# Ryo1011gd/ParticleMethod_FSI

Hardware: AMD Instinct MI355X
Metric: particle-steps/sec + achieved HBM GB/s, dam-break, 1/2/4/8 MI355X (higher is better)
Workload: dtype f64; 1 GPU; d1m: 3-D dam break (SURVEY 8d D1M, BASELINE configs[1]), 1397200 particles, ~1397200 per GPU; particles=1397200, dim=3, module=dam, parallelism=single

## Files before the change

include/mph_gpu.h:

```cpp
#ifndef MPH_GPU_H_INCLUDED
#define MPH_GPU_H_INCLUDED

#include <stddef.h>

#ifdef __cplusplus
extern "C" {
#endif

#define MPH_TYPE_COUNT 6
#define MPH_MAX_NEIGHBOR_COUNT 512
#define MPH_ABI_VERSION 6

typedef enum MphModule {
    MPH_MODULE_BAR = 0,
    MPH_MODULE_DAM = 1,
    MPH_MODULE_TUREK_HRON = 2,
    MPH_MODULE_ROLLING1 = 3,
    MPH_MODULE_HYDROELASTIC = 4,
    MPH_MODULE_NONE = 5
} MphModule;

typedef enum MphWallMotion {
    MPH_WALL_RIGID = 0,
    MPH_WALL_ROLLING = 1
// ... 227 lines not shown
    const char* unique_id128;
    mph_host_exchange_fn host_fn;
    void* host_user;
    int n_glob;
    const int* ids;
    const double* cuts;
} MphSlabOptions;
int mph_create_slab(MphCtx** ctx, const MphConfig* cfg, int n, const int* property, const double* pos,
                    const double* pos0, const double* vel, int device, const MphSlabOptions* opt);
int mph_slab_window(const MphConfig* cfg, int rank, int nranks, int axis, const double* cuts, double* out2);
int mph_dist_selftest(int device);
int mph_dist_info(const MphCtx* ctx, int* out8);
int mph_dist_overlap(const MphCtx* ctx, double* out5);
int mph_list_stats(MphCtx* ctx, double* mean, int* max);
int mph_list_layout(MphCtx* ctx, long long out6[6]);
int mph_neighbor_rows(MphCtx* ctx, int first, int count, int* counts, int* ids, long long ids_cap);
int mph_owned_count(const MphCtx* ctx);
int mph_owned_ids(MphCtx* ctx, int* out_ids);
int mph_slab_bounds(const MphConfig* cfg, int rank, int nranks, int axis, const double* cuts, double* out3);
int mph_slab_owner(const MphConfig* cfg, int nranks, int axis, const double* cuts, double c);

#ifdef __cplusplus
}
#endif
#endif
```

particlemethod_fsi_amd/csrc/mph_ctx.h:

```cpp
#pragma once

#include <hip/hip_runtime.h>

#include <cstdlib>
#include <string>
#include <thread>
#include <vector>

#include "mph_internal.h"
#include "mph_kernels.h"

struct MphDist {
    int rank = 0, nranks = 1, left = 0, right = 0;
    mph::SlabGeom g{};
    std::vector<double> cuts;
    int cap = 0;
    int n_own = 0;
    mph::DistLayout* lay = nullptr;
    mph::DistLayout* hlay = nullptr;
    int cap_sl = 0, cap_sr = 0, cap_rl = 0, cap_rr = 0;
    size_t region = 0;
    mph::Soa C;
    int* cls = nullptr;
    int* vidx = nullptr;
// ... 58 lines not shown
    std::vector<int> sl_s;
    int* order = nullptr;
    double *vir = nullptr, *vpres = nullptr;
    mph::StructDev Sd;
    std::vector<void*> allocs;
    mph::Launch L;
    bool mon_on = false;
    mph::MonitorDev mon;
    size_t mon_ring_cap = 0;
    int *mon_sorted = nullptr, *mon_map = nullptr;
    double* mon_probes = nullptr;
    long long mon_read = 0;
    double* sample_out = nullptr;
    size_t sample_cap = 0;
    bool a_current = false;
    MphDist* dist = nullptr;
};

#define MPH_HIP_OK(ctx, expr)                                                \
    do {                                                                     \
        hipError_t _e = (expr);                                              \
        if (_e != hipSuccess) return mph::ctx_hip_fail(ctx, _e, #expr);      \
    } while (0)

#define MPH_CK(expr)                   \
    do {                               \
        int _r = (expr);               \
        if (_r != MPH_OK) return _r;   \
    } while (0)

// ... 51 lines not shown
```

particlemethod_fsi_amd/csrc/mph_ctx.hip:

```cpp
#include <hip/hip_runtime.h>

#include <algorithm>
#include <chrono>
#include <cmath>
#include <cstdio>
#include <cstdlib>
#include <cstring>
#include <map>
#include <memory>
#include <string>
#include <vector>

#include "mph_ctx.h"
#include "mph_rows.h"

using namespace mph;

namespace mph {

int ctx_fail(MphCtx* c, int code, const std::string& msg)
{
    if (c) c->err = msg;
    return code;
}
// ... 30 lines not shown
    if (hs.overflow & 4)
        return ctx_fail(c, MPH_ERR_NONFINITE, "non-finite particle position (diverged state)");
    if (hs.overflow & 1)
        return ctx_fail(c, MPH_ERR_NEIGHBOR_OVERFLOW, "a particle has more than 512 neighbours");
    if (hs.overflow & 2) return ctx_fail(c, MPH_ERR_CAPACITY, "a particle moved past a neighbouring slab");
    if (hs.overflow & 64)
        return ctx_fail(c, MPH_ERR_HIP, "cell sort: histogram inconsistent with the keys (placement out of range)");
    return MPH_OK;
}

void ctx_fill_launch(MphCtx* c)
{
    Launch& L = c->L;
    set_uniforms(c->P);
    if (std::getenv("MPH_LIST_FULL") && std::atoi(std::getenv("MPH_LIST_FULL")) == 1) c->P.rlf = 3.0e38f;
    L.P = &c->P;
    L.stream = c->stream;
    const char* bm = std::getenv("MPH_XCD_BAL_MIN");
    L.xcd_bal_min = bm && *bm ? std::atoi(bm) : (1 << 20);
    L.S = &c->Sd;
}

int virial_full_lists(MphCtx* c)
{
    if (c->P.rlf >= 3.0e38f) return MPH_OK;
    DevParams Pf = c->P;
    Pf.rlf = 3.0e38f;
    Launch L = c->L;
    L.P = &Pf;
    L.xcd_bal_min = 0x7fffffff;
    launch_neighbors(L);
    MPH_HIP_OK(c, hipGetLastError());
    return MPH_OK;
}
}

namespace {

void enqueue_step(const Launch& L, bool last, hipEvent_t* ev = nullptr)
{
    if (ev) (void)hipEventRecord(ev[0], L.stream);
    launch_sort(L, 1);
    Launch La = L;
    if (!last) {
        La.dens_a = La.vstrain = La.divp = nullptr;
        if (!L.P->surface) La.gx = La.gy = La.gz = La.pa = nullptr;
    }
    if (ev) {
        launch_neighbors(La);
        (void)hipEventRecord(ev[1], L.stream);
        launch_pass_a(La);
    } else {
        launch_search_pass_a(La);
    }
    if (last) {
        launch_pass_b(L);
    } else {
        Launch Lb = L;
        Lb.force = nullptr;
        Lb.acc = nullptr;
        launch_pass_b(Lb);
    }
    launch_structure(L, last);
    if (ev) (void)hipEventRecord(ev[2], L.stream);
    if (L.mon) launch_monitor(L, *L.mon);
}

int capture(MphCtx* c, int steps, hipGraphExec_t* out, bool store_last = true)
{
    hipGraph_t g = nullptr;
    MPH_HIP_OK(c, hipStreamBeginCapture(c->stream, hipStreamCaptureModeThreadLocal));
    for (int k = 0; k < steps; ++k) enqueue_step(c->L, store_last && k == steps - 1);
    MPH_HIP_OK(c, hipStreamEndCapture(c->stream, &g));
    MPH_HIP_OK(c, hipGraphInstantiate(out, g, nullptr, nullptr, 0));
    MPH_HIP_OK(c, hipGraphDestroy(g));
// ... 448 lines not shown
    for (double* m : {D.F, D.E, D.S})
        MPH_HIP_OK(c, hipMemsetAsync(m, 0, sizeof(double) * 9 * nl, c->stream));
    MPH_HIP_OK(c, hipStreamSynchronize(c->stream));
    return MPH_OK;
}

static int init_first_sums(MphCtx* c)
{
    ctx_fill_launch(c);
    if (c->dist) {
        MPH_CK(dist_alloc(c));
        MPH_CK(dist_init(c));
    } else {
        launch_sort(c->L, 0);
        launch_search_pass_a(c->L);
    }
    MPH_HIP_OK(c, hipGetLastError());
    MPH_HIP_OK(c, hipStreamSynchronize(c->stream));
    DevState hs;
    MPH_HIP_OK(c, hipMemcpy(&hs, c->L.st, kStateHead, hipMemcpyDeviceToHost));
    return ctx_state_status(c, hs);
}

static int ctx_init(MphCtx* c, CreateArgs& a)
{
    MPH_CK(init_check_args(c, a));
    MPH_CK(init_host_state(c, a));
    MPH_CK(init_grid(c, a));
    MPH_CK(init_capacity(c, a));
    MPH_CK(init_alloc(c, a));
// ... 588 lines not shown
    for (long long t = 0; t < waves; ++t) {
        const int J = jump_count(R.hdr[t]);
        jumped += J > 0;
        jumps += J;
        max_jumps = std::max<long long>(max_jumps, J);
    }
    for (int s = 0; s < n; ++s) {
        const int rows = std::min(R.rows[s], kTileRows);
        gap_rows += rows - R.entries(s);
        max_rows = std::max<long long>(max_rows, rows);
    }
    out[0] = waves; out[1] = jumped; out[2] = jumps; out[3] = max_jumps; out[4] = gap_rows; out[5] = max_rows;
    return MPH_OK;
}

int mph_neighbor_rows(MphCtx* c, int first, int count, int* counts, int* ids, long long ids_cap)
{
    if (!c || first < 0 || count < 0 || !counts || (!ids && ids_cap > 0)) return MPH_ERR_ARG;
    MPH_CK(ctx_flush(c));
    if (c->dist) return ctx_fail(c, MPH_ERR_UNSUPPORTED, "mph_neighbor_rows: single contexts only");
    if ((long long)first + count > c->n) return ctx_fail(c, MPH_ERR_ARG, "mph_neighbor_rows: range past the particle count");
    if (!count) return 0;
    MPH_HIP_OK(c, hipSetDevice(c->device));
    const int n = c->n;
    if (c->P.rlf < 3.0e38f)
        return ctx_fail(c, MPH_ERR_UNSUPPORTED, "mph_neighbor_rows: the lists keep only the pairs within the passes' "
                                            "radius (create the context with MPH_LIST_FULL=1 for the reference's lists)");
    std::vector<int> id(n), nv(n);
    MPH_HIP_OK(c, hipMemcpy(id.data(), c->L.A.id, sizeof(int) * n, hipMemcpyDeviceToHost));
    MPH_HIP_OK(c, hipMemcpy(nv.data(), c->L.nbcount, sizeof(int) * n, hipMemcpyDeviceToHost));
// ... 251 lines not shown
```

particlemethod_fsi_amd/csrc/mph_device.h:

```cpp
#pragma once

#include <hip/hip_runtime.h>
#include <hip/hip_ext.h>

#include <climits>
#include <type_traits>

#include "mph_kernels.h"
#include "mph_params.h"

namespace mph {

__device__ __forceinline__ double mod_exact(double x, double w)
{
#pragma clang fp contract(off)
    return x - w * floor(x / w);
}

template <bool FAST>
__device__ __forceinline__ double image_exact(double d, double w, double hw, double w075)
{
#pragma clang fp contract(off)
    const double s = d + hw;
    double m;
// ... 56 lines not shown
__device__ __forceinline__ void rsqrt_pair(double r2, double& r, double& ir)
{
    double y = __builtin_amdgcn_rsq(r2);
    const double e = fma(-(r2 * y), y, 1.0);
    y = fma(0.5 * y, e, y);
    ir = y;
    r = r2 * y;
}

__device__ __forceinline__ int cell_id(const DevParams& P, double x, double y, double z)
{
    const int cx = cell_axis(x, P.corg[0], P.dw[0], P.ginv[0], P.gc[0]);
    const int cy = cell_axis(y, P.corg[1], P.dw[1], P.ginv[1], P.gc[1]);
    const int cz = P.dim == 3 ? cell_axis(z, P.corg[2], P.dw[2], P.ginv[2], P.gc[2]) : 0;
    return cell_index(P, cx, cy, cz);
}

__device__ __forceinline__ bool dev_is_struct(int t) { return t == 2 || t == 3; }
__device__ __forceinline__ bool dev_is_fluid(int t) { return t == 0 || t == 1; }
__device__ __forceinline__ bool dev_is_wall(int t) { return t == 4 || t == 5; }

__device__ __forceinline__ bool wave_search_interior(const DevParams& P, const DevState* st, bool live,
                                                     double x, double y, double z)
{
    const int occ = st->seam_occ[(st->seam_step - 1) & 1];
    const double v[3] = {x, y, z};
    bool in = true;
#pragma unroll
    for (int k = 0; k < 3; ++k) {
        if (k == 2 && P.dim == 2) break;
// ... 209 lines not shown
```

particlemethod_fsi_amd/csrc/mph_kernels.h:

```cpp
#pragma once

#include <hip/hip_runtime.h>

#include "mph_params.h"

namespace mph {

struct StructDev {
    int* orig = nullptr;
    int* slot_of = nullptr;
    int* bidx = nullptr;
    int n_own = 0;
    int n_inner = 0;
    int wo = 0, wi = 0;
    int* ocnt = nullptr;
    int* icnt = nullptr;
    int* eo_nb = nullptr;
    int* ei_nb = nullptr;
    double4* wx0 = nullptr;
    double* L = nullptr;
    double2* lame = nullptr;
    double* inv_rho = nullptr;
    int* clamp = nullptr;
    double4* x0 = nullptr;
// ... 52 lines not shown

struct Launch {
    const DevParams* P = nullptr;
    const DevTables* T = nullptr;
    DevState* st = nullptr;
    hipStream_t stream = nullptr;
    Profiler* prof = nullptr;
    Soa A, B;
    int* dst_of = nullptr;
    int *key = nullptr, *slot = nullptr, *tmp = nullptr, *cnt = nullptr, *start = nullptr, *bsum = nullptr;
    int *nbr = nullptr, *ncount = nullptr, *nbcount = nullptr;
    unsigned long long *lhdr = nullptr, *lgap = nullptr;
    int* wface = nullptr;
    VSrc vsrc;
    int xcd_bal_min = 1 << 20;
    double *pres = nullptr, *gx = nullptr, *gy = nullptr, *gz = nullptr, *pa = nullptr;
    double *dens_a = nullptr, *vstrain = nullptr, *divp = nullptr;
    double4 *fpart = nullptr;
    double4 *rec = nullptr;
    double4 *force = nullptr, *acc = nullptr;
    const StructDev* S = nullptr;
    const MonitorDev* mon = nullptr;
};

struct SampleDev {
    double origin[3], spacing[3];
    int count[3];
    int tile[3];
    int tiles[3];
    int mask;
// ... 51 lines not shown
```

particlemethod_fsi_amd/csrc/mph_list.h:

```cpp
#pragma once

#include "mph_device.h"

namespace mph {

#ifndef MPH_LB
#define MPH_LB 256
#endif
constexpr int kWB = MPH_LB / 64;
__device__ __forceinline__ int list_blocks(int n) { return (n + MPH_LB - 1) / MPH_LB; }

constexpr int kWaveCost = 16;

__device__ __forceinline__ int list_block(const DevState* st, int n, bool rev = false)
{
    const int nb = list_blocks(n);
    const int b = blockIdx.x;
    if (st) {
        const int* fr = st->xcd_frac;
        const int cap = gridDim.x >> 3;
        const int j = b & 7;
        bool ok = fr[0] == 0 && fr[8] == 65536;
        int lo = 0, mine_lo = 0, mine_c = 0;
        for (int x = 0; x < 8; ++x) {
            const int hi = (int)(((long long)fr[x + 1] * nb) >> 16);
            const int c = hi - lo;
            ok = ok && c >= 0 && c <= cap;
            if (x == j) { mine_lo = lo; mine_c = c; }
            lo = hi;
        }
        if (ok) {
            const int q = b >> 3;
            return q < mine_c ? mine_lo + (rev ? mine_c - 1 - q : q) : -1;
        }
    }
    if (b >= nb) return -1;
    if (!rev) return xcd_block(b, nb);
    const int xcd = b & 7, q = nb >> 3, r = nb & 7;
    const int lo = xcd < r ? xcd * (q + 1) : r * (q + 1) + (xcd - r) * q;
    const int cnt = q + (xcd < r ? 1 : 0);
    return lo + cnt - 1 - (b >> 3);
}

static inline int list_grid(int n)
{
    const int nb = blocks(n, MPH_LB);
    return (nb + nb / 4 + 15) / 8 * 8;
}

__device__ __forceinline__ void add_wave_work(DevState* st, int cnt, int i, int n)
{
    if (!st) return;
    int m = cnt;
    for (int o = 32; o; o >>= 1) m = max(m, __shfl_xor(m, o));
    const int tile = __builtin_amdgcn_readfirstlane(i >> 6);
    const int ntile = (n + 63) >> 6;
    if ((threadIdx.x & 63) == 0 && tile < ntile)
        atomicAdd(&st->seg_work[(int)(((long long)tile * kXcdSegs) / ntile)], m + kWaveCost);
}

__device__ __forceinline__ int nbr_entry(int j, int type) { return j | (type << kTypeShift); }
constexpr int kListKeep = 256 + (1 << 18), kListTotal = 1 << 18, kSoffMask = 0x3FFFF;
__device__ __forceinline__ int soff_total(int soff) { return (int)((unsigned)soff >> 18); }
__device__ __forceinline__ int soff_stored(int soff) { return (soff >> 8) & 0x3FF; }

__device__ __forceinline__ const int* ell_row(const int* nbr, int i)
{
    return nbr + (size_t)(i >> 6) * kTileStride + (i & 63);
}

__device__ __forceinline__ const int* ell_at(const int* row, int lane, int k)
{
    return row - lane + ell_slot(k, lane);
// ... 132 lines not shown
```

particlemethod_fsi_amd/csrc/mph_params.h:

```cpp
#pragma once
#include <cmath>

#include <cstddef>
#include <cstdint>

#include "../../include/mph_gpu.h"


namespace mph {

constexpr int kTypes = MPH_TYPE_COUNT;
constexpr int kMaxNeighbor = MPH_MAX_NEIGHBOR_COUNT;
constexpr int kTile = 64;
constexpr int kAlignRows = 128;
constexpr int kMaxJumps = 6;
#ifndef MPH_TILE_EXTRA
#define MPH_TILE_EXTRA kAlignRows
#endif
constexpr int kTileRows = kMaxNeighbor + MPH_TILE_EXTRA;
#ifndef MPH_TILE_PAD
#define MPH_TILE_PAD 1
#endif
constexpr int kTileStride = kTile * (kTileRows + MPH_TILE_PAD);
#if defined(__HIPCC__)
// ... 87 lines not shown
    for (int d = 0; d < 3; ++d) P.cwid[d] = 1.0 / P.ginv[d];
    P.rg_r2g = P.rg / P.r2g;
    double hwm = 0.0;
    for (int d = 0; d < 3; ++d) {
        P.cref[d] = P.dmin[d] + P.hw[d];
        hwm = P.hw[d] > hwm ? P.hw[d] : hwm;
    }
    const double rc = std::sqrt(P.rc2);
    const double delta = 2.0 * (2.0 * 1.7320508 * hwm * 1.1920929e-7 / rc) + 4.0e-6;
    P.rc2f_lo = (float)(P.rc2 * (1.0 - delta));
    P.rc2f_hi = (float)(P.rc2 * (1.0 + delta));
    const double rmax = std::fmax(std::fmax(P.ra, P.rg), std::fmax(P.rp, P.rv));
    P.rlf = (float)(rmax * rmax * (1.0 + delta));
}

constexpr int kXcdSegs = 4096;

struct DevState {
    double time;
    double wall_c[kTypes][3];
    double wall_vel[kTypes][3];
    double wall_omega[kTypes][3];
    double wall_rot[kTypes][3][3];
    int overflow;
    int pad0;
    int seam_occ[2];
    int seam_step;
    int seam_pad;
    int seg_work[kXcdSegs];
    int xcd_frac[9];
    int xcd_pad[3];
};
constexpr size_t kStateHead = offsetof(DevState, seg_work);

#if defined(__HIPCC__)
#define MPH_HD __host__ __device__
#else
#define MPH_HD
#endif

MPH_HD inline int jump_count(unsigned long long hdr) { return (int)(hdr >> 56); }
MPH_HD inline int gap_begin(unsigned long long gap, int k) { return (int)((gap >> (8 * k)) & 0xff); }
MPH_HD inline int gap_end(unsigned long long hdr, int k) { return (int)((hdr >> (8 * k)) & 0xff); }

#ifndef MPH_PA_EQR
#define MPH_PA_EQR 1
// ... 74 lines not shown
```

particlemethod_fsi_amd/csrc/mph_passes.hip:

```cpp
#include <cstdio>
#include <cstdlib>
#include <type_traits>

#include "mph_list.h"

namespace mph {

__device__ __forceinline__ void own_velocity(const Soa& A, int i, double& vx, double& vy, double& vz)
{
    const double2 b = A.p6[3 * (size_t)i + 1], c = A.p6[3 * (size_t)i + 2];
    vx = b.y; vy = c.x; vz = c.y;
}


struct PassA {
    double da = 0.0, g0 = 0.0, g1 = 0.0, g2 = 0.0, vs = 0.0, dv = 0.0;
    double s0 = 0.0, s1 = 0.0, s2 = 0.0, v0 = 0.0, v1 = 0.0, v2 = 0.0;
};

template <bool FORCE, bool EQR = false>
__device__ __forceinline__ void pass_a_term(const DevParams& P, const double* s_ratio, const double* s_mu, int ti,
                                            int tj, bool solid, double q0, double q1, double q2, double r2,
                                            double dvx, double dvy, double dvz, PassA& o)
{
// ... 163 lines not shown

#ifndef MPH_PA_WPE
#define MPH_PA_WPE 4
#endif
#if MPH_PA_WPE
#define MPH_PA_ATTR __attribute__((amdgpu_waves_per_eu(MPH_PA_WPE)))
#else
#define MPH_PA_ATTR
#endif
template <int DIM>
__global__ __launch_bounds__(MPH_LB) MPH_PA_ATTR void k_pass_a(DevParams P, const DevTables* __restrict__ T, Soa A,
                                                const int* __restrict__ nbr,
                                                const int* __restrict__ ncount,
                                                const unsigned long long* __restrict__ lhdr,
                                                const unsigned long long* __restrict__ lgap, PassAOut pout,
                                                const DevState* __restrict__ st)
{
    const int n = dev_n(P);
    const int lb = list_block(st, n, MPH_PASS_A_REV);
    if (lb < 0) return;
    __shared__ double s_ratio[kTypes * kTypes];
    __shared__ double s_mu[kTypes * kTypes];
    if (threadIdx.x < kTypes * kTypes) {
        s_ratio[threadIdx.x] = T->ratio[threadIdx.x];
        s_mu[threadIdx.x] = T->mu_ij[threadIdx.x] * (-P.cvis * P.cdv * P.vol);
    }
    __syncthreads();
    const int i = lb * blockDim.x + threadIdx.x;
    const bool live = i < n;
    const int ii = live ? i : n - 1;
    const double xi = A.x[ii], yi = A.y[ii], zi = A.z[ii];
    if (wave_all_ghosts(P, A, live, ii)) {
        if (live && pout.rec) rec_store(pout.rec, P.n, i, xi, yi, zi, 0.0);
// ... 302 lines not shown
        for (int v = 0; v < 3; ++v) o[3 * u + v] = S[u][v];
    vpres[i] = DIM == 2 ? -1.0 / 2.0 * (S[0][0] + S[1][1]) : -1.0 / 3.0 * (S[0][0] + S[1][1] + S[2][2]);
}


static PassAOut pass_a_out(const Launch& L)
{
    return PassAOut{L.pres, L.gx, L.gy, L.gz, L.pa, L.dens_a, L.vstrain, L.divp, L.fpart, L.rec};
}

void launch_pass_a(const Launch& L)
{
    const DevParams& P = *L.P;
    if (P.n == 0) return;
    by_dim(P.dim, [&](auto D) {
        launch(L.prof, "pass_a", L.stream, k_pass_a<decltype(D)::value>, dim3(list_grid(P.n)), dim3(MPH_LB), P, L.T,
               L.A, L.nbr, L.ncount, L.lhdr, L.lgap, pass_a_out(L), L.st);
    });
}

void launch_search_pass_a(const Launch& L)
{
    launch_neighbors(L);
    launch_pass_a(L);
}

static StructHook struct_hook(const Launch& L)
{
    StructHook h{};
    if (L.P->n_struct > 0 && L.S && L.S->slot_of) {
        h.slot_of = L.S->slot_of;
        h.sx = L.S->x;
// ... 4 lines not shown
    }
    return h;
}

void launch_pass_b(const Launch& L, int phase)
{
    const DevParams& P = *L.P;
    if (P.n == 0) return;
    if (P.surface && !(L.gx && L.gy && L.gz && L.pa)) {
        std::fprintf(stderr, "mph: launch_pass_b with surface tension needs GravityCenter/PressureA\n");
        std::abort();
    }
    auto go = [&](auto SURF) {
        by_dim(P.dim, [&](auto D) {
            launch(L.prof, phase == 2 ? "pass_b_face" : "pass_b", L.stream,
                   k_pass_b<decltype(SURF)::value, decltype(D)::value>, dim3(list_grid(P.n)), dim3(MPH_LB), P, L.T, L.A,
                   L.rec, L.fpart, L.gx, L.gy, L.gz, L.pa, L.nbr, L.ncount, L.lhdr, L.lgap, L.force, L.acc, L.B, phase,
                   L.wface, struct_hook(L), L.st);
        });
    };
    if (P.surface) go(std::true_type{});
    else go(std::false_type{});
}

void launch_virial(const Launch& L, const Soa& X, double* vir, double* vpres)
{
    const DevParams& P = *L.P;
    if (P.n == 0) return;
    by_dim(P.dim, [&](auto D) {
        launch(L.prof, "virial", L.stream, k_virial<decltype(D)::value>, dim3(blocks(P.n, 256)), dim3(256), P, L.T,
               L.A, X, L.pres, L.pa, L.gx, L.gy, L.gz, L.nbr, L.ncount, L.lhdr, L.lgap, vir, vpres);
// ... 5 lines not shown
```

particlemethod_fsi_amd/csrc/mph_search.hip:

```cpp
#include "mph_list.h"

#ifndef MPH_SB
#define MPH_SB 2
#endif
#ifndef MPH_LDS_CAP
#define MPH_LDS_CAP 176
#endif

namespace mph {

__device__ __forceinline__ void start_load2(__amdgpu_buffer_rsrc_t r, unsigned ob, unsigned oe, int& b, int& e)
{
    asm volatile("s_nop 4\n\tbuffer_load_dword %0, %2, %4, 0 offen\n\tbuffer_load_dword %1, %3, %4, 0 offen"
                 : "=&v"(b), "=&v"(e) : "v"(ob), "v"(oe), "s"(r) : "memory");
}
__device__ __forceinline__ void start_landed(int& a, int& b) { asm volatile("" : "+v"(a), "+v"(b)); }

__host__ __device__ constexpr int stage_d(int cap, int sb) { return (cap + sb + 2 + 1) & ~1; }
__host__ __device__ constexpr int stage_t(int cap, int sb) { return (cap + sb + 8 + 3) & ~3; }
__host__ __device__ constexpr int stage_words(int cap, int sb) { return 3 * stage_d(cap, sb) + stage_t(cap, sb) / 2; }


template <int DIM, int PERM> struct CellAxes {
    static constexpr int A0 = DIM == 3 ? order_axis(PERM, 0) : 0;
// ... 346 lines not shown
    return soff_total(soff);
}

__device__ __forceinline__ void slab_wave_flag(const DevParams& P, const Soa& A, int i, int n, int* wface)
{
    if (P.slab_axis < 0 || !wface) return;
    const bool live = i < n;
    const int ii = live ? i : n - 1;
    const bool own = live && A.id[ii] >= 0;
    const double c = P.slab_axis == 0 ? A.x[ii] : (P.slab_axis == 1 ? A.y[ii] : A.z[ii]);
    const bool inner = c - P.slab_lo > P.slab_h && P.slab_hi - c > P.slab_h;
    const bool face = !__all(!own || inner);
    if ((threadIdx.x & 63) == 0) wface[i >> 6] = face ? 1 : 0;
}

template <int DIM, int PERM>
__device__ __forceinline__ int neighbors_body(const DevParams& P, const Soa& A, const int* start, int* nbr,
                                               int* ncount, int* nbcount, unsigned long long* lhdr,
                                               unsigned long long* lgap, DevState* st, double* stage, int i)
{
    const int n = dev_n(P);
    const bool live = i < n;
    const int ii = live ? i : n - 1;
    const int tile = __builtin_amdgcn_readfirstlane(i >> 6);
    if (tile * kTile >= n) return 0;
    if (wave_all_ghosts(P, A, live, ii)) {
        if (live) ncount[i] = 0;
        if (live) nbcount[i] = 0;
        if ((threadIdx.x & 63) == 0) lhdr[tile] = 0;
        return 0;
// ... 12 lines not shown
    } else {
        if (own)
            cnt = scan_candidates<DIM, PERM>(P, A, start, i, xi, yi, zi, cx, cy, cz, out);
        stored = cnt;
        if ((threadIdx.x & 63) == 0) lhdr[tile] = 0;
    }
    if (live) ncount[i] = stored;
    if (live) nbcount[i] = cnt;
    if (cnt > kMaxNeighbor) atomicOr(&st->overflow, 1);
    return stored;
}

#ifndef MPH_NB_WPE
#define MPH_NB_WPE 8
#endif
template <int DIM, int PERM>
__global__ __launch_bounds__(MPH_LB) __attribute__((amdgpu_waves_per_eu(MPH_NB_WPE))) void k_neighbors(
    DevParams P, Soa A, const int* __restrict__ start, int* __restrict__ nbr, int* __restrict__ ncount,
    int* __restrict__ nbcount, unsigned long long* __restrict__ lhdr, unsigned long long* __restrict__ lgap,
    DevState* __restrict__ st, int* __restrict__ wface, int bal)
{
    const int n = dev_n(P);
    if ((int)blockIdx.x >= list_blocks(n)) return;
    const int tb = xcd_block(blockIdx.x, list_blocks(n));
    __shared__ __attribute__((aligned(16))) double stage[kWB][stage_words(MPH_LDS_CAP, MPH_SB)];
    const int i = tb * blockDim.x + threadIdx.x;
    slab_wave_flag(P, A, i, n, wface);
    const int cnt = neighbors_body<DIM, PERM>(P, A, start, nbr, ncount, nbcount, lhdr, lgap, st,
                                              stage[__builtin_amdgcn_readfirstlane(threadIdx.x >> 6)], i);
    if (bal) add_wave_work(st, cnt, i, n);
}


void launch_neighbors(const Launch& L)
{
    const DevParams& P = *L.P;
    if (P.n == 0) return;
    const int bal = P.n >= L.xcd_bal_min;
    by_dim(P.dim, [&](auto D) {
        constexpr int DIM = decltype(D)::value;
        auto go = [&](auto PERM) {
            launch(L.prof, "neighbors", L.stream, k_neighbors<DIM, decltype(PERM)::value>, dim3(blocks(P.n, MPH_LB)),
                   dim3(MPH_LB), P, L.A, L.start, L.nbr, L.ncount, L.nbcount, L.lhdr, L.lgap, L.st, L.wface, bal);
        };
        if constexpr (DIM == 3) {
            switch (P.perm) {
            case 1: go(Int<1>{}); break;
            case 2: go(Int<2>{}); break;
            case 3: go(Int<3>{}); break;
            case 4: go(Int<4>{}); break;
            default: go(Int<0>{}); break;
            }
        } else {
            go(Int<0>{});
        }
    });
}

// ... 2 lines not shown
```

particlemethod_fsi_amd/csrc/mph_sort.hip:

```cpp
#include "mph_device.h"

namespace mph {


__device__ __forceinline__ int seam_bits(const DevParams& P, double x, double y, double z)
{
    const double v[3] = {x, y, z};
    int b = 0;
#pragma unroll
    for (int k = 0; k < 3; ++k) {
        if (k == 2 && P.dim == 2) break;
        if ((P.seam_always >> k) & 1) continue;
        b |= (v[k] < P.inner_lo[k] ? 1 : 0) << (2 * k);
        b |= (v[k] > P.inner_hi[k] ? 2 : 0) << (2 * k);
    }
    return b;
}

constexpr int kScanThreads = 256;
#ifndef MPH_SCAN_ITEMS
#define MPH_SCAN_ITEMS 16
#endif
constexpr int kScanItems = MPH_SCAN_ITEMS;
constexpr int kScanBlock = kScanThreads * kScanItems;
__host__ __device__ inline int bsum_stride(int ncell) { return ncell / kScanBlock + 2; }
static_assert(kScanBlock == 4096, "mph_ctx.hip sizes the bsum buffer for 4096-cell blocks");

template <int T>
__device__ __forceinline__ void xcd_split_block(DevState* st)
{
    constexpr int R = kXcdSegs / T;
    static_assert(kXcdSegs % T == 0, "whole runs per thread");
    __shared__ long long s[T];
    const int t = threadIdx.x;
    long long sum = 0;
    for (int r = 0; r < R; ++r) sum += max(st->seg_work[t * R + r], 0);
    s[t] = sum;
    __syncthreads();
    for (int o = 1; o < T; o <<= 1) {
        const long long v = t >= o ? s[t - o] : 0;
        __syncthreads();
        s[t] += v;
        __syncthreads();
    }
    const long long tot = s[T - 1];
    int* fr = st->xcd_frac;
    if (tot < 8) {
        if (t < 9) fr[t] = 8192 * t;
    } else {
        for (int x = 1; x < 8; ++x) {
            const long long tgt = tot * x / 8;
            long long prev = t ? s[t - 1] : 0;
            if (!(prev < tgt && s[t] >= tgt)) continue;
            for (int r = 0; r < R; ++r) {
                const int w = max(st->seg_work[t * R + r], 0);
                if (w > 0 && prev < tgt && prev + w >= tgt) {
                    const double f = (t * R + r + (double)(tgt - prev) / (double)w) / kXcdSegs;
                    fr[x] = min(65536, max(0, (int)(f * 65536.0 + 0.5)));
                }
                prev += w;
            }
        }
        if (t == 0) {
            fr[0] = 0;
            fr[8] = 65536;
        }
    }
    __syncthreads();
    for (int r = 0; r < R; ++r) st->seg_work[t * R + r] = 0;
}

__global__ __launch_bounds__(256) void k_prep(DevParams P, const DevState* __restrict__ st, Soa C,
                                              int* __restrict__ key, int* __restrict__ slot,
                                              int* __restrict__ cnt, int mode, VSrc vs)
{
    const int p = blockIdx.x * blockDim.x + threadIdx.x;
    const int n = dev_n(P);
    Soa B = C;
    bool mig = false;
    const int b = p < n ? vsrc_entry(vs, C, p, B, mig) : p;
    {
        const bool live = p < n;
        int k = -1 - (int)(threadIdx.x & 63);
        int occ = 0;
        if (live) {
            double x = B.x[b], y = B.y[b], z = B.z[b];
            if (mode == 1) move_and_wrap(P, st, B, b, x, y, z);
            if (!isfinite(x + y + z)) atomicOr(const_cast<int*>(&st->overflow), 4);
            k = cell_id(P, x, y, z);
            key[p] = k;
            occ = seam_bits(P, x, y, z);
        }
        const int lane = threadIdx.x & 63;
        const int kprev = __shfl_up(k, 1, 64);
        const bool head = lane == 0 || kprev != k;
        const unsigned long long heads = __ballot(head);
        const unsigned long long upto = lane == 63 ? ~0ull : ((2ull << lane) - 1ull);
        const int hl = 63 - __clzll(heads & upto);
        const unsigned long long above = heads & ~upto;
        const int next = above ? __ffsll((long long)above) - 1 : 64;
        int base = 0;
        if (live && head) base = atomicAdd(&cnt[k], next - lane);
        base = __shfl(base, hl, 64);
        if (live) slot[p] = base + (lane - hl);
        __shared__ int s_occ;
// ... 157 lines not shown
    if (p >= n) return;
    const int d = start[key[p]] + slot[p];
    if ((unsigned)d >= (unsigned)n) {
        atomicOr(&st->overflow, 64);
        return;
    }
    tmp[d] = p;
}

__global__ __launch_bounds__(256) void k_rank_scatter(DevParams P, const int* __restrict__ key,
                                                      const int* __restrict__ start,
                                                      const int* __restrict__ tmp, Soa C, Soa A,
                                                      int* __restrict__ rank_of, int* __restrict__ dst_of,
                                                      int mode, VSrc vs, DevState* __restrict__ st, int split)
{
    if (split && blockIdx.x == 0) xcd_split_block<256>(st);
    const int p = blockIdx.x * blockDim.x + threadIdx.x;
    if (p >= dev_n(P)) return;
    const int k = key[p];
    const int s = start[k], e = start[k + 1];
    int r = 0;
    for (int q = s; q < e; ++q) r += tmp[q] < p;
    const int dst = s + r;
    Soa B;
    bool mig;
    const int b = vsrc_entry(vs, C, p, B, mig);
    A.x[dst] = B.x[b];
    A.y[dst] = B.y[b];
    A.z[dst] = B.z[b];
    if (dst_of && mode == 0) {
        A.vx[dst] = B.vx[b];
// ... 17 lines not shown
                 Profiler* prof)
{
    const int nb = blocks(ncell, kScanBlock);
    const int top = nb <= kScanFusedTop;
    launch(prof, "scan_reduce", stream, k_scan_reduce, dim3(nb), dim3(kScanThreads), cnt, ncell, bsum);
    if (!top) launch(prof, "scan_top", stream, k_scan_top, dim3(1), dim3(1024), bsum, nb);
    launch(prof, "scan_down", stream, k_scan_down, dim3(nb), dim3(kScanThreads), cnt, ncell, bsum, start, total,
           n_dev, top);
}

void launch_sort(const Launch& L, int mode)
{
    const DevParams& P = *L.P;
    const int n = P.n;
    if (n == 0) return;
    const int split = n >= L.xcd_bal_min;
    const dim3 g(blocks(n, 256)), b(256);
    launch(L.prof, "prep", L.stream, k_prep, g, b, P, L.st, L.B, L.key, L.slot, L.cnt, mode, L.vsrc);
    launch_scan(L.cnt, P.ncell, L.bsum, L.start, n, P.n_dev, L.stream, L.prof);
    launch(L.prof, "place", L.stream, k_place, g, b, P, L.st, L.key, L.slot, L.start, L.tmp, mode);
    launch(L.prof, "rank_scatter", L.stream, k_rank_scatter, g, b, P, L.key, L.start, L.tmp, L.B, L.A,
           nullptr , L.dst_of, mode,
           L.vsrc, L.st, split);
}

}
```

particlemethod_fsi_amd/solver.py:

```python
from __future__ import annotations

import ctypes
import os
import subprocess

import numpy as np

from . import mphio

PKG_DIR = os.path.dirname(os.path.abspath(__file__))
LIB_DIR = os.path.join(PKG_DIR, "lib")
LIB_PATH = os.environ.get("MPH_GPU_LIB") or os.path.join(LIB_DIR, "libmph_gpu.so")
CSRC_DIR = os.path.join(PKG_DIR, "csrc")

FIELDS = {
    "Position": (0, 3, np.float64), "InitialPosition": (1, 3, np.float64),
    "Velocity": (2, 3, np.float64), "Force": (3, 3, np.float64),
    "Acceleration": (4, 3, np.float64), "GravityCenter": (5, 3, np.float64),
    "PressureP": (6, 1, np.float64), "PressureA": (7, 1, np.float64),
    "DensityA": (8, 1, np.float64), "VolStrainP": (9, 1, np.float64),
    "DivergenceP": (10, 1, np.float64), "Mass": (11, 1, np.float64), "Kappa": (12, 1, np.float64),
    "Lambda": (13, 1, np.float64), "Mu": (14, 1, np.float64),
    "NeighborCount": (15, 1, np.int32), "InitialStructureNeighborCount": (16, 1, np.int32),
    "Property": (17, 1, np.int32), "DeformGradient": (18, 9, np.float64),
# ... 10 lines not shown

EXPORTED_SYMBOLS = [
    "mph_config_default", "mph_read_data_file", "mph_read_grid_header", "mph_read_grid_particles",
    "mph_write_prof_arrays", "mph_write_vtk_arrays", "mph_create", "mph_step", "mph_synchronize",
    "mph_get", "mph_set", "mph_particle_count", "mph_time", "mph_get_scalars", "mph_write_prof",
    "mph_write_vtk", "mph_last_error", "mph_destroy", "mph_profile_steps", "mph_profile_graphs", "mph_neighbor_stats",
    "mph_dist_unique_id", "mph_create_dist", "mph_owned_count", "mph_derive_scalars",
    "mph_structure_init", "mph_create_dist_host", "mph_owned_ids", "mph_slab_bounds",
    "mph_slab_owner", "mph_dist_selftest", "mph_compute_virial",
    "mph_config_sizeof", "mph_write_vtk_async", "mph_output_wait", "mph_write_grid_binary",
    "mph_write_vtu_arrays", "mph_write_vtu", "mph_velocity_profile_arrays",
    "mph_set_initial_velocity_profile", "mph_dist_info", "mph_create_slab", "mph_slab_window",
    "mph_list_stats", "mph_abi_version", "mph_phase_timing", "mph_phase_times",
    "mph_set_step_batching", "mph_neighbor_rows", "mph_dist_overlap", "mph_list_layout",
    "mph_monitor_configure", "mph_monitor_sample_doubles", "mph_monitor_read",
    "mph_sample_grid", "mph_sample_grid_timed", "mph_write_vti_arrays",
]

ABI_VERSION = 6

HOST_EXCHANGE_FN = ctypes.CFUNCTYPE(ctypes.c_int, ctypes.c_void_p, ctypes.c_void_p, ctypes.c_size_t,
                                    ctypes.c_void_p, ctypes.c_size_t, ctypes.c_void_p, ctypes.c_size_t,
                                    ctypes.c_void_p, ctypes.c_size_t)


class MphSlabOptions(ctypes.Structure):
    _fields_ = [("rank", ctypes.c_int), ("nranks", ctypes.c_int), ("axis", ctypes.c_int),
                ("unique_id128", ctypes.c_char_p), ("host_fn", HOST_EXCHANGE_FN),
                ("host_user", ctypes.c_void_p), ("n_glob", ctypes.c_int), ("ids", ctypes.c_void_p),
                ("cuts", ctypes.c_void_p)]

# ... 120 lines not shown
        "mph_list_stats": (ip, [vp, vp, vp]),
        "mph_create_slab": (ip, [ctypes.POINTER(vp), cfgp, ip, vp, vp, vp, vp, ip, ctypes.POINTER(MphSlabOptions)]),
        "mph_slab_window": (ip, [cfgp, ip, ip, ip, vp, vp]),
        "mph_phase_timing": (ip, [vp, ip]),
        "mph_phase_times": (ip, [vp, vp]),
        "mph_set_step_batching": (ip, [vp, ip]),
        "mph_neighbor_rows": (ip, [vp, ip, ip, vp, vp, ctypes.c_longlong]),
        "mph_dist_overlap": (ip, [vp, vp]),
        "mph_list_layout": (ip, [vp, vp]),
        "mph_monitor_configure": (ip, [vp, ctypes.POINTER(MphMonitorConfig)]),
        "mph_monitor_sample_doubles": (ip, [vp]),
        "mph_monitor_read": (ctypes.c_longlong, [vp, vp, ctypes.c_longlong, ctypes.POINTER(ctypes.c_longlong)]),
        "mph_sample_grid": (ip, [vp, ctypes.POINTER(MphSampleGrid), vp]),
        "mph_sample_grid_timed": (ip, [vp, ctypes.POINTER(MphSampleGrid), vp, ctypes.POINTER(ctypes.c_double), vp]),
        "mph_write_vti_arrays": (ip, [ctypes.c_char_p, ctypes.POINTER(MphSampleGrid), vp]),
    }
    optional = {"mph_phase_timing", "mph_phase_times", "mph_set_step_batching", "mph_neighbor_rows",
                "mph_dist_overlap", "mph_profile_graphs", "mph_list_stats", "mph_list_layout",
                "mph_monitor_configure", "mph_monitor_sample_doubles", "mph_monitor_read",
                "mph_sample_grid", "mph_sample_grid_timed", "mph_write_vti_arrays"}
    for name, (res, args) in sig.items():
        if name in optional and not hasattr(L, name):
            continue
        f = getattr(L, name)
        f.restype = res
        f.argtypes = args
    accept = {ABI_VERSION} | {int(v) for v in os.environ.get("MPH_ABI_ACCEPT", "").split(",") if v.strip()}
    if L.mph_abi_version() not in accept:
        raise ImportError("%s has C ABI version %d, these bindings expect %d (rebuild the library)"
                          % (LIB_PATH, L.mph_abi_version(), ABI_VERSION))
    if L.mph_config_sizeof() != ctypes.sizeof(mphio.MphConfig):
        raise ImportError("MphConfig layout mismatch between %s and mphio.MphConfig" % LIB_PATH)
    _lib = L
    return L

# ... 316 lines not shown
        _check(self._L.mph_owned_ids(self._h, out.ctypes.data), self._h)
        return out[:k].copy()

    def list_stats(self):
        m = ctypes.c_double()
        x = ctypes.c_int()
        _check(self._L.mph_list_stats(self._h, ctypes.byref(m), ctypes.byref(x)), self._h)
        return m.value, x.value

    def list_layout(self) -> dict:
        a = np.zeros(6, np.int64)
        _check(self._L.mph_list_layout(self._h, a.ctypes.data), self._h)
        keys = ["waves", "waves_jumped", "jumps", "max_jumps", "gap_rows", "max_rows"]
        return {k: int(v) for k, v in zip(keys, a)}

    def neighbor_rows(self, first: int = 0, count: int | None = None):
        if count is None:
            count = self.n - first
        counts = np.zeros(count, np.int32)
        cap = max(1, count * 128)
        while True:
            ids = np.zeros(cap, np.int32)
            r = self._L.mph_neighbor_rows(self._h, int(first), int(count), counts.ctypes.data, ids.ctypes.data, cap)
            need = int(np.minimum(counts, 512).sum()) if r == -1 else 0
            if r == -1 and need > cap:
                cap = need
                continue
            _check(r, self._h)
            break
        offsets = np.concatenate([[0], np.cumsum(np.minimum(counts, 512))]).astype(np.int64)
# ... 41 lines not shown
```

Measured before the change: 1.363 billion particle-steps/s.

## Skip neighbor search for wall waves far from any fluid via coarse occupancy map

Adds a coarse occupancy bitmap (4x4x4 cells) that the sort prep kernel marks for every non-wall particle and pass_a clears. In the neighbor kernel, a wave made entirely of wall particles whose search box touches no occupied coarse cell gets empty lists and skips the search. Load balancing now tracks separate list-work and search-work segments with their own XCD split, and the list kernels get enlarged grids. This removes search and pass work for the many idle wall particles in dam-break, at the cost of extra atomics, an extra map write per particle and extra DevState fields.

```diff
diff --git a/include/mph_gpu.h b/include/mph_gpu.h
--- a/include/mph_gpu.h
+++ b/include/mph_gpu.h
@@ -265,6 +265,7 @@
 int mph_dist_overlap(const MphCtx* ctx, double* out5);
 int mph_list_stats(MphCtx* ctx, double* mean, int* max);
 int mph_list_layout(MphCtx* ctx, long long out6[6]);
+int mph_idle_wall_stats(MphCtx* ctx, long long out2[2]);
 int mph_neighbor_rows(MphCtx* ctx, int first, int count, int* counts, int* ids, long long ids_cap);
 int mph_owned_count(const MphCtx* ctx);
 int mph_owned_ids(MphCtx* ctx, int* out_ids);
diff --git a/particlemethod_fsi_amd/csrc/mph_ctx.h b/particlemethod_fsi_amd/csrc/mph_ctx.h
--- a/particlemethod_fsi_amd/csrc/mph_ctx.h
+++ b/particlemethod_fsi_amd/csrc/mph_ctx.h
@@ -96,6 +96,7 @@
     double* sample_out = nullptr;
     size_t sample_cap = 0;
     bool a_current = false;
+    bool lazy_walls = false;
     MphDist* dist = nullptr;
 };
 
diff --git a/particlemethod_fsi_amd/csrc/mph_ctx.hip b/particlemethod_fsi_amd/csrc/mph_ctx.hip
--- a/particlemethod_fsi_amd/csrc/mph_ctx.hip
+++ b/particlemethod_fsi_amd/csrc/mph_ctx.hip
@@ -68,6 +68,7 @@
     Launch& L = c->L;
     set_uniforms(c->P);
     if (std::getenv("MPH_LIST_FULL") && std::atoi(std::getenv("MPH_LIST_FULL")) == 1) c->P.rlf = 3.0e38f;
+    c->lazy_walls = !c->dist && !(std::getenv("MPH_LAZY_WALLS") && std::atoi(std::getenv("MPH_LAZY_WALLS")) == 0);
     L.P = &c->P;
     L.stream = c->stream;
     const char* bm = std::getenv("MPH_XCD_BAL_MIN");
@@ -94,8 +95,9 @@
 void enqueue_step(const Launch& L, bool last, hipEvent_t* ev = nullptr)
 {
     if (ev) (void)hipEventRecord(ev[0], L.stream);
-    launch_sort(L, 1);
     Launch La = L;
+    La.lazy = !last && L.cmap && !L.mon;
+    launch_sort(La, 1);
     if (!last) {
         La.dens_a = La.vstrain = La.divp = nullptr;
         if (!L.P->surface) La.gx = La.gy = La.gz = La.pa = nullptr;
@@ -113,6 +115,7 @@
         Launch Lb = L;
         Lb.force = nullptr;
         Lb.acc = nullptr;
+        Lb.lazy = La.lazy;
         launch_pass_b(Lb);
     }
     launch_structure(L, last);
@@ -591,6 +594,12 @@
     } else {
         launch_sort(c->L, 0);
         launch_search_pass_a(c->L);
+        if (c->lazy_walls) {
+            const size_t mb = coarse_map_bytes(c->P.gc);
+            MPH_CK(ctx_dalloc(c, &c->L.cmap, mb));
+            MPH_HIP_OK(c, hipMemsetAsync(c->L.cmap, 0, mb, c->stream));
+            c->L.cmap_bytes = (int)mb;
+        }
     }
     MPH_HIP_OK(c, hipGetLastError());
     MPH_HIP_OK(c, hipStreamSynchronize(c->stream));
@@ -1209,6 +1218,25 @@
     return MPH_OK;
 }
 
+int mph_idle_wall_stats(MphCtx* c, long long out[2])
+{
+    if (!c || !out) return MPH_ERR_ARG;
+    MPH_CK(ctx_flush(c));
+    MPH_HIP_OK(c, hipSetDevice(c->device));
+    MPH_HIP_OK(c, hipStreamSynchronize(c->stream));
+    unsigned long long steps = 0;
+    std::vector<unsigned> seg(kXcdSegs);
+    const char* st = reinterpret_cast<const char*>(c->L.st);
+    MPH_HIP_OK(c, hipMemcpy(&steps, st + offsetof(DevState, lazy_steps), sizeof(steps), hipMemcpyDeviceToHost));
+    MPH_HIP_OK(c, hipMemcpy(seg.data(), st + offsetof(DevState, idle_waves), sizeof(unsigned) * kXcdSegs,
+                            hipMemcpyDeviceToHost));
+    long long idle = 0;
+    for (unsigned v : seg) idle += v;
+    out[0] = idle;
+    out[1] = (long long)steps;
+    return MPH_OK;
+}
+
 int mph_neighbor_rows(MphCtx* c, int first, int count, int* counts, int* ids, long long ids_cap)
 {
     if (!c || first < 0 || count < 0 || !counts || (!ids && ids_cap > 0)) return MPH_ERR_ARG;
diff --git a/particlemethod_fsi_amd/csrc/mph_device.h b/particlemethod_fsi_amd/csrc/mph_device.h
--- a/particlemethod_fsi_amd/csrc/mph_device.h
+++ b/particlemethod_fsi_amd/csrc/mph_device.h
@@ -94,6 +94,11 @@
     const int cy = cell_axis(y, P.corg[1], P.dw[1], P.ginv[1], P.gc[1]);
     const int cz = P.dim == 3 ? cell_axis(z, P.corg[2], P.dw[2], P.ginv[2], P.gc[2]) : 0;
     return cell_index(P, cx, cy, cz);
+}
+
+__device__ __forceinline__ int coarse_index(const DevParams& P, int qx, int qy, int qz)
+{
+    return (qx * coarse_cells(P.gc[1]) + qy) * coarse_cells(P.gc[2]) + qz;
 }
 
 __device__ __forceinline__ bool dev_is_struct(int t) { return t == 2 || t == 3; }
diff --git a/particlemethod_fsi_amd/csrc/mph_kernels.h b/particlemethod_fsi_amd/csrc/mph_kernels.h
--- a/particlemethod_fsi_amd/csrc/mph_kernels.h
+++ b/particlemethod_fsi_amd/csrc/mph_kernels.h
@@ -90,6 +90,9 @@
     int* wface = nullptr;
     VSrc vsrc;
     int xcd_bal_min = 1 << 20;
+    unsigned char* cmap = nullptr;
+    int cmap_bytes = 0;
+    bool lazy = false;
     double *pres = nullptr, *gx = nullptr, *gy = nullptr, *gz = nullptr, *pa = nullptr;
     double *dens_a = nullptr, *vstrain = nullptr, *divp = nullptr;
     double4 *fpart = nullptr;
diff --git a/particlemethod_fsi_amd/csrc/mph_list.h b/particlemethod_fsi_amd/csrc/mph_list.h
--- a/particlemethod_fsi_amd/csrc/mph_list.h
+++ b/particlemethod_fsi_amd/csrc/mph_list.h
@@ -12,12 +12,11 @@
 
 constexpr int kWaveCost = 16;
 
-__device__ __forceinline__ int list_block(const DevState* st, int n, bool rev = false)
+__device__ __forceinline__ int list_block(const int* fr, int n, bool rev = false)
 {
     const int nb = list_blocks(n);
     const int b = blockIdx.x;
-    if (st) {
-        const int* fr = st->xcd_frac;
+    if (fr) {
         const int cap = gridDim.x >> 3;
         const int j = b & 7;
         bool ok = fr[0] == 0 && fr[8] == 65536;
@@ -41,22 +40,30 @@
     const int cnt = q + (xcd < r ? 1 : 0);
     return lo + cnt - 1 - (b >> 3);
 }
-
-static inline int list_grid(int n)
+__device__ __forceinline__ int list_block(const DevState* st, int n, bool rev = false)
+{
+    return list_block(st ? st->xcd_frac : nullptr, n, rev);
+}
+
+static inline int list_grid(int n, bool lazy = false)
 {
     const int nb = blocks(n, MPH_LB);
-    return (nb + nb / 4 + 15) / 8 * 8;
-}
-
-__device__ __forceinline__ void add_wave_work(DevState* st, int cnt, int i, int n)
-{
-    if (!st) return;
+    return ((lazy ? 3 * nb : nb + nb / 4) + 15) / 8 * 8;
+}
+
+constexpr int kSearchCost = 16, kIdleCost = 2;
+
+__device__ __forceinline__ void add_wave_work(int* seg, int cnt, int i, int n, int* sseg = nullptr, bool idle = false)
+{
     int m = cnt;
     for (int o = 32; o; o >>= 1) m = max(m, __shfl_xor(m, o));
     const int tile = __builtin_amdgcn_readfirstlane(i >> 6);
     const int ntile = (n + 63) >> 6;
-    if ((threadIdx.x & 63) == 0 && tile < ntile)
-        atomicAdd(&st->seg_work[(int)(((long long)tile * kXcdSegs) / ntile)], m + kWaveCost);
+    if ((threadIdx.x & 63) == 0 && tile < ntile) {
+        const int r = (int)(((long long)tile * kXcdSegs) / ntile);
+        atomicAdd(&seg[r], m + kWaveCost);
+        if (sseg) atomicAdd(&sseg[r], idle ? kIdleCost : kSearchCost);
+    }
 }
 
 __device__ __forceinline__ int nbr_entry(int j, int type) { return j | (type << kTypeShift); }
diff --git a/particlemethod_fsi_amd/csrc/mph_params.h b/particlemethod_fsi_amd/csrc/mph_params.h
--- a/particlemethod_fsi_amd/csrc/mph_params.h
+++ b/particlemethod_fsi_amd/csrc/mph_params.h
@@ -125,6 +125,17 @@
     P.rlf = (float)(rmax * rmax * (1.0 + delta));
 }
 
+constexpr int kCoarseShift = 2;
+#if defined(__HIPCC__)
+__host__ __device__
+#endif
+constexpr inline int coarse_cells(int g) { return (g + (1 << kCoarseShift) - 1) >> kCoarseShift; }
+inline size_t coarse_map_bytes(const int gc[3])
+{
+    const size_t b = (size_t)coarse_cells(gc[0]) * coarse_cells(gc[1]) * coarse_cells(gc[2]);
+    return (b + 15) & ~(size_t)15;
+}
+
 constexpr int kXcdSegs = 4096;
 
 struct DevState {
@@ -141,6 +152,12 @@
     int seg_work[kXcdSegs];
     int xcd_frac[9];
     int xcd_pad[3];
+    unsigned long long lazy_steps;
+    unsigned idle_waves[kXcdSegs];
+    int seg_lwork[kXcdSegs];
+    int seg_swork[kXcdSegs];
+    int xcd_sfrac[9];
+    int xcd_spad[3];
 };
 constexpr size_t kStateHead = offsetof(DevState, seg_work);
 
diff --git a/particlemethod_fsi_amd/csrc/mph_passes.hip b/particlemethod_fsi_amd/csrc/mph_passes.hip
--- a/particlemethod_fsi_amd/csrc/mph_passes.hip
+++ b/particlemethod_fsi_amd/csrc/mph_passes.hip
@@ -201,9 +201,13 @@
                                                 const int* __restrict__ ncount,
                                                 const unsigned long long* __restrict__ lhdr,
                                                 const unsigned long long* __restrict__ lgap, PassAOut pout,
-                                                const DevState* __restrict__ st)
+                                                const DevState* __restrict__ st,
+                                                unsigned char* __restrict__ cmap, int cmap_bytes)
 {
     const int n = dev_n(P);
+    if (cmap)
+        for (int q = blockIdx.x * MPH_LB + threadIdx.x; q * 16 < cmap_bytes; q += gridDim.x * MPH_LB)
+            reinterpret_cast<int4*>(cmap)[q] = make_int4(0, 0, 0, 0);
     const int lb = list_block(st, n, MPH_PASS_A_REV);
     if (lb < 0) return;
     __shared__ double s_ratio[kTypes * kTypes];
@@ -536,8 +540,9 @@
     const DevParams& P = *L.P;
     if (P.n == 0) return;
     by_dim(P.dim, [&](auto D) {
-        launch(L.prof, "pass_a", L.stream, k_pass_a<decltype(D)::value>, dim3(list_grid(P.n)), dim3(MPH_LB), P, L.T,
-               L.A, L.nbr, L.ncount, L.lhdr, L.lgap, pass_a_out(L), L.st);
+        launch(L.prof, "pass_a", L.stream, k_pass_a<decltype(D)::value>,
+               dim3(list_grid(P.n, L.lazy && P.n >= L.xcd_bal_min)), dim3(MPH_LB), P, L.T,
+               L.A, L.nbr, L.ncount, L.lhdr, L.lgap, pass_a_out(L), L.st, L.lazy ? L.cmap : nullptr, L.cmap_bytes);
     });
 }
 
@@ -572,7 +577,8 @@
     auto go = [&](auto SURF) {
         by_dim(P.dim, [&](auto D) {
             launch(L.prof, phase == 2 ? "pass_b_face" : "pass_b", L.stream,
-                   k_pass_b<decltype(SURF)::value, decltype(D)::value>, dim3(list_grid(P.n)), dim3(MPH_LB), P, L.T, L.A,
+                   k_pass_b<decltype(SURF)::value, decltype(D)::value>,
+                   dim3(list_grid(P.n, L.lazy && P.n >= L.xcd_bal_min)), dim3(MPH_LB), P, L.T, L.A,
                    L.rec, L.fpart, L.gx, L.gy, L.gz, L.pa, L.nbr, L.ncount, L.lhdr, L.lgap, L.force, L.acc, L.B, phase,
                    L.wface, struct_hook(L), L.st);
         });
diff --git a/particlemethod_fsi_amd/csrc/mph_search.hip b/particlemethod_fsi_amd/csrc/mph_search.hip
--- a/particlemethod_fsi_amd/csrc/mph_search.hip
+++ b/particlemethod_fsi_amd/csrc/mph_search.hip
@@ -384,6 +384,48 @@
     if ((threadIdx.x & 63) == 0) wface[i >> 6] = face ? 1 : 0;
 }
 
+template <int DIM>
+__device__ __forceinline__ bool wave_idle_walls(const DevParams& P, const Soa& A, const unsigned char* cmap,
+                                                DevState* st, int* ncount, int* nbcount,
+                                                unsigned long long* lhdr, int i, int n)
+{
+    static_assert(kContigReach <= kReach, "the box is widened by kReach on every axis");
+    static_assert(2 * kReach < 2 << kCoarseShift, "a lane's box spans at most 3 coarse cells per axis");
+    const int tile = __builtin_amdgcn_readfirstlane(i >> 6);
+    if (tile * kTile >= n) return false;
+    const bool live = i < n;
+    int ii = live ? i : n - 1;
+    asm volatile("" : "+v"(ii));
+    if (!__all(!live || dev_is_wall(A.type[ii]))) return false;
+    const double xi = A.x[ii], yi = A.y[ii], zi = A.z[ii];
+    if (!wave_search_interior(P, st, live, xi, yi, zi)) return false;
+    const int cx = cell_axis(xi, P.corg[0], P.dw[0], P.ginv[0], P.gc[0]);
+    const int cy = cell_axis(yi, P.corg[1], P.dw[1], P.ginv[1], P.gc[1]);
+    const int cz = DIM == 3 ? cell_axis(zi, P.corg[2], P.dw[2], P.ginv[2], P.gc[2]) : 0;
+    const int ax = max(cx - kReach, 0) >> kCoarseShift, bx = min(cx + kReach, P.gc[0] - 1) >> kCoarseShift;
+    const int ay = max(cy - kReach, 0) >> kCoarseShift, by = min(cy + kReach, P.gc[1] - 1) >> kCoarseShift;
+    const int az = DIM == 3 ? max(cz - kReach, 0) >> kCoarseShift : 0;
+    const int bz = DIM == 3 ? min(cz + kReach, P.gc[2] - 1) >> kCoarseShift : 0;
+    const int ny = coarse_cells(P.gc[1]), nz = coarse_cells(P.gc[2]);
+    int hit = 0;
+#pragma unroll 1
+    for (int kx = 0; kx < 3; ++kx) {
+#pragma unroll 1
+        for (int ky = 0; ky < 3; ++ky) {
+            const unsigned char* row = cmap + (min(ax + kx, bx) * ny + min(ay + ky, by)) * nz;
+            hit |= row[az] | row[min(az + 1, bz)] | row[bz];
+        }
+    }
+    if (__ballot(hit != 0)) return false;
+    if (live) ncount[i] = 0;
+    if (live) nbcount[i] = 0;
+    if ((threadIdx.x & 63) == 0) {
+        lhdr[tile] = 0;
+        atomicAdd(&st->idle_waves[(int)(((long long)tile * kXcdSegs) / ((n + 63) >> 6))], 1u);
+    }
+    return true;
+}
+
 template <int DIM, int PERM>
 __device__ __forceinline__ int neighbors_body(const DevParams& P, const Soa& A, const int* start, int* nbr,
                                                int* ncount, int* nbcount, unsigned long long* lhdr,
@@ -426,21 +468,34 @@
 #ifndef MPH_NB_WPE
 #define MPH_NB_WPE 8
 #endif
-template <int DIM, int PERM>
+template <int DIM, int PERM, bool LAZY>
 __global__ __launch_bounds__(MPH_LB) __attribute__((amdgpu_waves_per_eu(MPH_NB_WPE))) void k_neighbors(
     DevParams P, Soa A, const int* __restrict__ start, int* __restrict__ nbr, int* __restrict__ ncount,
     int* __restrict__ nbcount, unsigned long long* __restrict__ lhdr, unsigned long long* __restrict__ lgap,
-    DevState* __restrict__ st, int* __restrict__ wface, int bal)
-{
+    DevState* __restrict__ st, int* __restrict__ wface, int bal, const unsigned char* __restrict__ cmap_arg)
+{
+    const unsigned char* cmap = LAZY ? cmap_arg : nullptr;
     const int n = dev_n(P);
-    if ((int)blockIdx.x >= list_blocks(n)) return;
-    const int tb = xcd_block(blockIdx.x, list_blocks(n));
+    if (cmap && blockIdx.x == 0 && threadIdx.x == 0) st->lazy_steps += 1;
+    int tb;
+    if (cmap && bal) {
+        tb = list_block(st->xcd_sfrac, n);
+        if (tb < 0) return;
+    } else {
+        if ((int)blockIdx.x >= list_blocks(n)) return;
+        tb = xcd_block(blockIdx.x, list_blocks(n));
+    }
     __shared__ __attribute__((aligned(16))) double stage[kWB][stage_words(MPH_LDS_CAP, MPH_SB)];
     const int i = tb * blockDim.x + threadIdx.x;
     slab_wave_flag(P, A, i, n, wface);
-    const int cnt = neighbors_body<DIM, PERM>(P, A, start, nbr, ncount, nbcount, lhdr, lgap, st,
-                                              stage[__builtin_amdgcn_readfirstlane(threadIdx.x >> 6)], i);
-    if (bal) add_wave_work(st, cnt, i, n);
+    const bool idle = cmap && wave_idle_walls<DIM>(P, A, cmap, st, ncount, nbcount, lhdr, i, n);
+    const int cnt = idle ? 0
+                         : neighbors_body<DIM, PERM>(P, A, start, nbr, ncount, nbcount, lhdr, lgap, st,
+                                                     stage[__builtin_amdgcn_readfirstlane(threadIdx.x >> 6)], i);
+    if (bal) {
+        if (cmap) add_wave_work(st->seg_lwork, cnt, i, n, st->seg_swork, idle);
+        else add_wave_work(st->seg_work, cnt, i, n);
+    }
 }
 
 
@@ -449,11 +504,18 @@
     const DevParams& P = *L.P;
     if (P.n == 0) return;
     const int bal = P.n >= L.xcd_bal_min;
+    const bool lazy = L.lazy && L.cmap;
     by_dim(P.dim, [&](auto D) {
         constexpr int DIM = decltype(D)::value;
         auto go = [&](auto PERM) {
-            launch(L.prof, "neighbors", L.stream, k_neighbors<DIM, decltype(PERM)::value>, dim3(blocks(P.n, MPH_LB)),
-                   dim3(MPH_LB), P, L.A, L.start, L.nbr, L.ncount, L.nbcount, L.lhdr, L.lgap, L.st, L.wface, bal);
+            if (lazy)
+                launch(L.prof, "neighbors", L.stream, k_neighbors<DIM, decltype(PERM)::value, true>,
+                       dim3(bal ? list_grid(P.n, true) : blocks(P.n, MPH_LB)), dim3(MPH_LB), P, L.A, L.start, L.nbr,
+                       L.ncount, L.nbcount, L.lhdr, L.lgap, L.st, L.wface, bal, L.cmap);
+            else
+                launch(L.prof, "neighbors", L.stream, k_neighbors<DIM, decltype(PERM)::value, false>,
+                       dim3(blocks(P.n, MPH_LB)), dim3(MPH_LB), P, L.A, L.start, L.nbr, L.ncount, L.nbcount, L.lhdr,
+                       L.lgap, L.st, L.wface, bal, nullptr);
         };
         if constexpr (DIM == 3) {
             switch (P.perm) {
diff --git a/particlemethod_fsi_amd/csrc/mph_sort.hip b/particlemethod_fsi_amd/csrc/mph_sort.hip
--- a/particlemethod_fsi_amd/csrc/mph_sort.hip
+++ b/particlemethod_fsi_amd/csrc/mph_sort.hip
@@ -27,14 +27,14 @@
 static_assert(kScanBlock == 4096, "mph_ctx.hip sizes the bsum buffer for 4096-cell blocks");
 
 template <int T>
-__device__ __forceinline__ void xcd_split_block(DevState* st)
+__device__ __forceinline__ void xcd_split_block(int* seg, int* fr)
 {
     constexpr int R = kXcdSegs / T;
     static_assert(kXcdSegs % T == 0, "whole runs per thread");
     __shared__ long long s[T];
     const int t = threadIdx.x;
     long long sum = 0;
-    for (int r = 0; r < R; ++r) sum += max(st->seg_work[t * R + r], 0);
+    for (int r = 0; r < R; ++r) sum += max(seg[t * R + r], 0);
     s[t] = sum;
     __syncthreads();
     for (int o = 1; o < T; o <<= 1) {
@@ -44,7 +44,6 @@
         __syncthreads();
     }
     const long long tot = s[T - 1];
-    int* fr = st->xcd_frac;
     if (tot < 8) {
         if (t < 9) fr[t] = 8192 * t;
     } else {
@@ -53,7 +52,7 @@
             long long prev = t ? s[t - 1] : 0;
             if (!(prev < tgt && s[t] >= tgt)) continue;
             for (int r = 0; r < R; ++r) {
-                const int w = max(st->seg_work[t * R + r], 0);
+                const int w = max(seg[t * R + r], 0);
                 if (w > 0 && prev < tgt && prev + w >= tgt) {
                     const double f = (t * R + r + (double)(tgt - prev) / (double)w) / kXcdSegs;
                     fr[x] = min(65536, max(0, (int)(f * 65536.0 + 0.5)));
@@ -67,12 +66,13 @@
         }
     }
     __syncthreads();
-    for (int r = 0; r < R; ++r) st->seg_work[t * R + r] = 0;
-}
-
-__global__ __launch_bounds__(256) void k_prep(DevParams P, const DevState* __restrict__ st, Soa C,
-                                              int* __restrict__ key, int* __restrict__ slot,
-                                              int* __restrict__ cnt, int mode, VSrc vs)
+    for (int r = 0; r < R; ++r) seg[t * R + r] = 0;
+    __syncthreads();
+}
+
+__global__ __launch_bounds__(256) __attribute__((amdgpu_waves_per_eu(8))) void k_prep(
+    DevParams P, const DevState* __restrict__ st, Soa C, int* __restrict__ key, int* __restrict__ slot,
+    int* __restrict__ cnt, int mode, VSrc vs, unsigned char* __restrict__ cmap)
 {
     const int p = blockIdx.x * blockDim.x + threadIdx.x;
     const int n = dev_n(P);
@@ -87,8 +87,13 @@
             double x = B.x[b], y = B.y[b], z = B.z[b];
             if (mode == 1) move_and_wrap(P, st, B, b, x, y, z);
             if (!isfinite(x + y + z)) atomicOr(const_cast<int*>(&st->overflow), 4);
-            k = cell_id(P, x, y, z);
+            const int cx = cell_axis(x, P.corg[0], P.dw[0], P.ginv[0], P.gc[0]);
+            const int cy = cell_axis(y, P.corg[1], P.dw[1], P.ginv[1], P.gc[1]);
+            const int cz = P.dim == 3 ? cell_axis(z, P.corg[2], P.dw[2], P.ginv[2], P.gc[2]) : 0;
+            k = cell_index(P, cx, cy, cz);
             key[p] = k;
+            if (cmap && !dev_is_wall(B.type[b]))
+                cmap[coarse_index(P, cx >> kCoarseShift, cy >> kCoarseShift, cz >> kCoarseShift)] = 1;
             occ = seam_bits(P, x, y, z);
         }
         const int lane = threadIdx.x & 63;
@@ -276,7 +281,10 @@
                                                       int* __restrict__ rank_of, int* __restrict__ dst_of,
                                                       int mode, VSrc vs, DevState* __restrict__ st, int split)
 {
-    if (split && blockIdx.x == 0) xcd_split_block<256>(st);
+    if (split && blockIdx.x == 0) {
+        xcd_split_block<256>(split == 2 ? st->seg_lwork : st->seg_work, st->xcd_frac);
+        if (split == 2) xcd_split_block<256>(st->seg_swork, st->xcd_sfrac);
+    }
     const int p = blockIdx.x * blockDim.x + threadIdx.x;
     if (p >= dev_n(P)) return;
     const int k = key[p];
@@ -324,9 +332,10 @@
     const DevParams& P = *L.P;
     const int n = P.n;
     if (n == 0) return;
-    const int split = n >= L.xcd_bal_min;
+    const int split = n >= L.xcd_bal_min ? (L.lazy ? 2 : 1) : 0;
     const dim3 g(blocks(n, 256)), b(256);
-    launch(L.prof, "prep", L.stream, k_prep, g, b, P, L.st, L.B, L.key, L.slot, L.cnt, mode, L.vsrc);
+    launch(L.prof, "prep", L.stream, k_prep, g, b, P, L.st, L.B, L.key, L.slot, L.cnt, mode, L.vsrc,
+           L.lazy ? L.cmap : nullptr);
     launch_scan(L.cnt, P.ncell, L.bsum, L.start, n, P.n_dev, L.stream, L.prof);
     launch(L.prof, "place", L.stream, k_place, g, b, P, L.st, L.key, L.slot, L.start, L.tmp, mode);
     launch(L.prof, "rank_scatter", L.stream, k_rank_scatter, g, b, P, L.key, L.start, L.tmp, L.B, L.A,
diff --git a/particlemethod_fsi_amd/solver.py b/particlemethod_fsi_amd/solver.py
--- a/particlemethod_fsi_amd/solver.py
+++ b/particlemethod_fsi_amd/solver.py
@@ -48,7 +48,7 @@
     "mph_list_stats", "mph_abi_version", "mph_phase_timing", "mph_phase_times",
     "mph_set_step_batching", "mph_neighbor_rows", "mph_dist_overlap", "mph_list_layout",
     "mph_monitor_configure", "mph_monitor_sample_doubles", "mph_monitor_read",
-    "mph_sample_grid", "mph_sample_grid_timed", "mph_write_vti_arrays",
+    "mph_sample_grid", "mph_sample_grid_timed", "mph_write_vti_arrays", "mph_idle_wall_stats",
 ]
 
 ABI_VERSION = 6
@@ -199,11 +199,12 @@
         "mph_sample_grid": (ip, [vp, ctypes.POINTER(MphSampleGrid), vp]),
         "mph_sample_grid_timed": (ip, [vp, ctypes.POINTER(MphSampleGrid), vp, ctypes.POINTER(ctypes.c_double), vp]),
         "mph_write_vti_arrays": (ip, [ctypes.c_char_p, ctypes.POINTER(MphSampleGrid), vp]),
+        "mph_idle_wall_stats": (ip, [vp, vp]),
     }
     optional = {"mph_phase_timing", "mph_phase_times", "mph_set_step_batching", "mph_neighbor_rows",
                 "mph_dist_overlap", "mph_profile_graphs", "mph_list_stats", "mph_list_layout",
                 "mph_monitor_configure", "mph_monitor_sample_doubles", "mph_monitor_read",
-                "mph_sample_grid", "mph_sample_grid_timed", "mph_write_vti_arrays"}
+                "mph_sample_grid", "mph_sample_grid_timed", "mph_write_vti_arrays", "mph_idle_wall_stats"}
     for name, (res, args) in sig.items():
         if name in optional and not hasattr(L, name):
             continue
@@ -550,6 +551,12 @@
         keys = ["waves", "waves_jumped", "jumps", "max_jumps", "gap_rows", "max_rows"]
         return {k: int(v) for k, v in zip(keys, a)}
 
+    def idle_wall_stats(self) -> dict:
+        a = np.zeros(2, np.int64)
+        if hasattr(self._L, "mph_idle_wall_stats"):
+            _check(self._L.mph_idle_wall_stats(self._h, a.ctypes.data), self._h)
+        return {"idle_wave_steps": int(a[0]), "lazy_steps": int(a[1])}
+
     def neighbor_rows(self, first: int = 0, count: int | None = None):
         if count is None:
             count = self.n - first
```

After: 1.468 billion particle-steps/s, median of 6. +7.7%, better.
